# Corleno/Nonstationary_Multivariate_Gaussian_Process

Measured on AMD Instinct MI355X. Metric: log-posterior evals/sec (N=2048, D=3 nonseparable GP), higher is better.
Workload: dtype f64

## Files before the change

nonstationary_multivariate_gaussian_process_amd/csrc/nmgp_api.hip:

```cpp
#include <cstdarg>

#include "nmgp_internal.h"

using namespace nmgpk;

enum {
    SC_LOGDET = 0,
    SC_QUAD = 1,
    SC_PRIORQ = 2,
    SC_TRACE = 40,
    SC_OUT = 48,
    SC_MISC = 56,
    SC_COUNT = 128
};

int nmgp_fail(nmgp_ctx* ctx, int code, const char* fmt, ...) {
    char buf[1024];
    va_list ap;
    va_start(ap, fmt);
    vsnprintf(buf, sizeof(buf), fmt, ap);
    va_end(ap);
    if (ctx) ctx->err = buf;
    return code;
}
// ... 774 lines not shown
    PriorFactor pf;
    pf.alpha = alpha;
    pf.beta = beta;
    const size_t N = c->N, B = (size_t)c->batch / c->b_cps;
    pf.ld = (int)(((N + 15) / 16) * 16);
    NMGP_TRY(nmgp_dev_alloc(c, &pf.L, B * (size_t)pf.ld * N));
    if (nmgp_dev_alloc(c, &pf.logdet, B) != 0) {
        hipFree(pf.L);
        return NMGP_E_NOMEM;
    }
    int* info;
    HIP_TRY(c, hipMalloc((void**)&info, B * sizeof(int)));
    hipMemsetAsync(info, 0, B * sizeof(int), c->stream);
    rbf_cov_sym(c->stream, c->b_x, c->N, alpha, beta, pf.L, pf.ld, false, (int)B);
    nmgp_potrf(c, pf.L, pf.ld, c->N, 0, 0, info, (int)B, (long long)pf.ld * N, 1, 1);
    half_logdet(c->stream, pf.L, pf.ld, c->N, pf.logdet, (int)B);
    std::vector<int> hi(B);
    hipMemcpyAsync(hi.data(), info, B * sizeof(int), hipMemcpyDeviceToHost, c->stream);
    hipError_t e = hipStreamSynchronize(c->stream);
    hipFree(info);
    int bad = 0;
    for (size_t b = 0; b < B; ++b)
        if (hi[b] != 0 && bad == 0) bad = hi[b];
    if (e != hipSuccess || bad != 0) {
        hipFree(pf.L);
        hipFree(pf.logdet);
        if (e != hipSuccess) return nmgp_fail(c, NMGP_E_HIP, "batched prior factorisation failed (%s)", hipGetErrorString(e));
        return nmgp_fail(c, bad, "GP prior covariance RBF(alpha=%g, beta=%g)+jitter of a subject is not positive definite "
                         "(leading minor %d)", alpha, beta, bad);
    }
    c->b_priors.push_back(pf);
    *out = &c->b_priors.back();
    return 0;
}

static int batch_grad_alloc(nmgp_ctx* c) {
    if (c->b_grad_ready) return 0;
    const size_t N = c->N, T = c->T, n = c->n, P = (size_t)c->P_svc, B = c->batch;
    const size_t ld2 = nmgp_ld(2 * n + 2);
    const size_t NJ = (N + 63) / 64;
    NMGP_TRY(nmgp_dev_alloc(c, &c->b_S2, B * ld2 * n));
    NMGP_TRY(nmgp_dev_alloc(c, &c->b_Sinv, B * n * n));
    NMGP_TRY(nmgp_dev_alloc(c, &c->b_alpha, B * n));
    NMGP_TRY(nmgp_dev_alloc(c, &c->b_part, B * std::max(NJ * N * (T + 1), (size_t)n * ((n + 255) / 256))));
    NMGP_TRY(nmgp_dev_alloc(c, &c->b_grad, B * P));
    NMGP_TRY(nmgp_dev_alloc(c, &c->b_R2, N * B * (1 + T)));
    NMGP_TRY(nmgp_dev_alloc(c, &c->b_tr, B * 2));
    c->b_grad_ready = true;
    return 0;
}

static bool schur_selected(const nmgp_ctx* c, int want_grad) {
    if (want_grad || c->M < 2 || c->svc_schur == 0) return false;
    return true;
}

static int svc_batch_value_schur(nmgp_ctx* c, const double* xs, int xstride, const double* ys, long long ystride, int cps) {
    const int N = c->N, M = c->M, B = c->batch, n1 = (M - 1) * N;
    const long long P = c->P_svc;
    const int xpad = (N + 1) & 1, xoffA = N + 1 + xpad;
    const int ldA = (int)nmgp_ld((size_t)2 * N + 2), ldP = (int)nmgp_ld((size_t)n1 + 1);
    auto r64 = [](size_t v) { return (v + 63) / 64 * 64; };
    const size_t offP = r64((size_t)ldA * N), offPart = r64(offP + (size_t)ldP * n1);
    const size_t need = r64(offPart + (size_t)N * ((N + 255) / 256));
    const size_t bsS = nmgp_ld((size_t)c->n + 1) * (size_t)c->n;
    double* base = c->b_S;
    size_t bsz = bsS;
    if (need > bsS) {
        if (c->b_schur_stride != need) {
            NMGP_TRY(nmgp_dev_alloc(c, &c->b_schur, (size_t)B * need));
            c->b_schur_stride = need;
        }
        base = c->b_schur;
        bsz = need;
    }
    const long long bs = (long long)bsz;
    double* A = base;
    double* Sp = base + offP;
    double* part = base + offPart;
    double* w = c->b_z;
    double* w1 = c->b_z + (size_t)B * N;
    const double* tse = c->b_pars + (P - 1);
    hipStream_t s = c->stream;
    HIP_TRY(c, hipMemsetAsync(c->b_info2, 0, (size_t)B * sizeof(int), s));
    {
        StageScope sp(c, NMGP_STAGE_COV);
        svc_prep(s, c->b_pars, N, M, c->b_ell, c->b_Lv, B);
        int r = svc_schur_a(s, xs, c->b_ell, c->b_Lv, tse, ys, A, ldA, xpad, N, M, B, bs, xstride, ystride, cps);
        if (r) return nmgp_fail(c, r, "unsupported number of outputs M=%d", M);
    }
    {
        StageScope sp(c, NMGP_STAGE_CHOL);
        nmgp_potrf(c, A, ldA, N, 1 + xpad, N, c->b_info, B, bs, 1);
    }
    {
        StageScope sp(c, NMGP_STAGE_SOLVE);
        get_row(s, A, ldA, N, w, N, B, bs, N);
        tri_gemv_upper(s, A + xoffA, ldA, N, w, c->b_u, part, B, bs, bs);
    }
    {
        StageScope sp(c, NMGP_STAGE_REDUCE);
        chol_logdet_quad(s, A, ldA, N, w, c->b_scal + 2, c->b_scal + 3, B, bs, 16);
    }
    {
        StageScope sp(c, NMGP_STAGE_INVERSE);
        const SchurEpi e{xs, c->b_ell, c->b_Lv, tse, ys, c->b_u, Sp, ldP, N, xstride, cps, ystride, bs};
        int r = syrk_schur(s, A + xoffA, ldA, N, M, B, e);
        if (r) return nmgp_fail(c, r, "unsupported number of outputs M=%d", M);
    }
    {
        StageScope sp(c, NMGP_STAGE_CHOL);
        nmgp_potrf(c, Sp, ldP, n1, 1, 0, c->b_info2, B, bs, 1);
    }
    {
        StageScope sp(c, NMGP_STAGE_SOLVE);
        get_row(s, Sp, ldP, n1, w1, n1, B, bs, n1);
    }
    {
        StageScope sp(c, NMGP_STAGE_REDUCE);
        chol_logdet_quad(s, Sp, ldP, n1, w1, c->b_scal + 4, c->b_scal + 5, B, bs, 16);
        svc_schur_combine(s, c->b_Lv, N, M, c->b_scal, 16, c->b_info, c->b_info2, B);
    }
    return 0;
}

extern "C" int nmgp_svc_batch_eval(nmgp_ctx* c, const double hyper[8], int prior, int want_grad) {
    if (!c) return NMGP_E_NULL;
    if (!hyper) return nmgp_fail(c, NMGP_E_NULL, "hyper must not be NULL");
    if (c->batch <= 0) return nmgp_fail(c, NMGP_E_STATE, "nmgp_svc_batch_alloc must be called first");
    HIP_TRY(c, hipSetDevice(c->device));
    const int N = c->N, M = c->M, T = c->T, n = c->n, B = c->batch;
    const long long P = c->P_svc;
    c->b_traj_ready = false;
    if (want_grad) NMGP_TRY(batch_grad_alloc(c));
    const int xpad = (n + 1) & 1, xoff = n + 1 + xpad;
    const int ld = want_grad ? (int)nmgp_ld((size_t)2 * n + 2) : (int)nmgp_ld((size_t)n + 1);
    double* S = want_grad ? c->b_S2 : c->b_S;
    const long long bs = (long long)ld * n;
    const double mu_l = hyper[0], al_l = hyper[1], be_l = hyper[2], mu_L = hyper[3], al_L = hyper[4], be_L = hyper[5];
    const double a = hyper[6], b = hyper[7];
    hipStream_t s = c->stream;
    const bool multi = c->b_multi;
    const int cps = multi ? c->b_cps : 1;
    const double* xs = multi ? c->b_x : c->d_x;
    const int xstride = multi ? N : 0;
    PriorFactor *pl = nullptr, *pL = nullptr;
    if (multi) {
        NMGP_TRY(get_batch_prior(c, al_l, be_l, &pl));
        NMGP_TRY(get_batch_prior(c, al_L, be_L, &pL));
        NMGP_TRY(get_batch_prior(c, al_l, be_l, &pl));
    } else {
        NMGP_TRY(nmgp_get_prior(c, al_l, be_l, &pl));
        NMGP_TRY(nmgp_get_prior(c, al_L, be_L, &pL));
        NMGP_TRY(nmgp_get_prior(c, al_l, be_l, &pl));
    }
    HIP_TRY(c, hipMemsetAsync(c->b_info, 0, (size_t)B * sizeof(int), s));
    if (nmgp_poison()) HIP_TRY(c, hipMemsetAsync(c->b_scal, 0xFF, (size_t)B * 16 * sizeof(double), s));
    PriorStreamScope ps(c);
    if (schur_selected(c, want_grad)) {
        NMGP_TRY(svc_batch_value_schur(c, xs, xstride, multi ? c->b_y : c->d_y, multi ? n : 0, cps));
    } else {
        {
            StageScope sp(c, NMGP_STAGE_COV);
            svc_prep(s, c->b_pars, N, M, c->b_ell, c->b_Lv, B);
            int r = svc_cov_build(s, xs, c->b_ell, c->b_Lv, c->b_pars + (P - 1), S, ld, N, M, false, B, bs, xstride, cps);
            if (r) return nmgp_fail(c, r, "unsupported number of outputs M=%d", M);
        }
        {
            StageScope sp(c, NMGP_STAGE_CHOL);
            set_row(s, S, ld, n, multi ? c->b_y : c->d_y, n, B, bs, multi ? n : 0, cps);
            if (want_grad) identity_rows(s, S, ld, n + 1, n, xpad, B, bs);
            nmgp_potrf(c, S, ld, n, want_grad ? 1 + xpad : 1, want_grad ? n : 0, c->b_info, B, bs, 1);
        }
        {
            StageScope sp(c, NMGP_STAGE_SOLVE);
            get_row(s, S, ld, n, c->b_z, n, B, bs, n);
            if (want_grad) {
                tri_gemv_upper(s, S + xoff, (int)ld, n, c->b_z, c->b_alpha, c->b_part, (int)B, bs,
                               (long long)n * ((n + 255) / 256));
            }
        }
        {
            StageScope sp(c, NMGP_STAGE_REDUCE);
            chol_logdet_quad(s, S, ld, n, c->b_z, c->b_scal, c->b_scal + 1, B, bs, 16);
        }
    }
    {
        NmgpStage sp(c, NMGP_STAGE_PRIOR, ps.sp, 0.0, 0.0);
        const double one = 1.0;
// ... 810 lines not shown
```

nonstationary_multivariate_gaussian_process_amd/csrc/nmgp_chol.hip:

```cpp
#include "nmgp_internal.h"
#include <cstring>

namespace nmgpk {

static inline int cdiv_c(long long a, long long b) { return (int)((a + b - 1) / b); }

typedef double v4d __attribute__((ext_vector_type(4)));

#define SY_BM 128
#define SY_BK 16
#define SY_LD (SY_BM + 16)
#define SY_SB 8

__device__ __forceinline__ int clamp_row_pair(int r, int rows) {
    int rc = r < rows - 1 ? r : rows - 2;
    return rc < 0 ? 0 : rc;
}

__device__ __forceinline__ double fast_recip(double p) {
    double x = __builtin_amdgcn_rcp(p);
    double e = fma(-p, x, 1.0);
    x = fma(x, e, x);
    e = fma(-p, x, 1.0);
    x = fma(x, e, x);
// ... 115 lines not shown
                svc_schur_value<M>(sigma2, a, b, r == c, Lr, il2, Lc, kv, nai, gcb);
        }
    }
}

constexpr int svc_gstride(int M) { return M + 2; }

template <int M>
__device__ __forceinline__ void svc_schur_gtable(const SchurEpi& e, double* lds, int row0, int col0, int tid) {
    constexpr int T = M * (M + 1) / 2, GS = svc_gstride(M);
    if constexpr (M <= 4) {
        double* gt = lds + 8 * SCHUR_PATCH;
        if (tid < 256) {
            const int loc = tid < 128 ? col0 + tid : row0 + tid - 128;
            if (loc < e.N) {
                const double sigma2 = exp(e.tse[0]);
                const double* Lc = e.Lv + (size_t)loc * T;
                const double l00 = Lc[0];
#pragma unroll
                for (int b = 1; b < M; ++b) gt[tid * GS + b - 1] = sigma2 * Lc[b * (b + 1) / 2] / (l00 * l00);
                gt[tid * GS + M - 1] = 1.0 / (l00 * l00);
                gt[tid * GS + M] = e.x[loc];
                gt[tid * GS + M + 1] = e.ell[loc];
            }
        }
        __syncthreads();
    }
}

template <int M>
__device__ __forceinline__ void svc_schur_patch(const SchurEpi& e, double* P, const double* lds, int i0, int j0, int row0, int col0,
                                                int lane) {
    constexpr int T_ = M * (M + 1) / 2, GS = svc_gstride(M);
    constexpr int QU = M <= 3 ? 2 : 1;
    const int N = e.N;
    const size_t Ns = (size_t)N;
    const double sigma2 = exp(e.tse[0]);
    const double* gt = lds + 8 * SCHUR_PATCH;
    const int lo = lane & 31, hi = lane >> 5;
    __builtin_amdgcn_wave_barrier();
#pragma unroll
    for (int pass = 0; pass < 2; ++pass) {
        if (pass == 1 && M == 2) break;
        const int r = (pass == 0 ? i0 : j0) + lo;
        if (r < N) {
            const double* __restrict__ Lr = e.Lv + (size_t)r * T_;
            const double xr = e.x[r], lr = e.ell[r];
            const double xr2 = xr * xr, lr2 = lr * lr;
            const double l00 = Lr[0];
            const double il2 = 1.0 / (l00 * l00);
#pragma unroll QU
            for (int q = 0; q < 16; ++q) {
                const int o = 2 * q + hi;
                const int il = pass == 0 ? lo : o, jl = pass == 0 ? o : lo;
                const int c = (pass == 0 ? j0 : i0) + o;
                if (pass == 0 ? (c > r || c >= N) : (c <= r || c >= N)) continue;
                const double* gc = gt + (pass == 0 ? c - col0 : 128 + c - row0) * GS;
                if (pass == 1 && M == 3) {
                    e.S[(size_t)c * e.ld + (Ns + r)] = P[il * 33 + jl];
                    continue;
                }
                const double xc = M <= 4 ? gc[M] : e.x[c], lc = M <= 4 ? gc[M + 1] : e.ell[c];
                const double dist = (xr2 + xc * xc) - 2.0 * (xr * xc);
                const double Aa = lr2 + lc * lc;
                double kv = sqrt(2.0 * (lr * lc) / Aa) * exp(-dist / Aa);
                if (r == c) kv = NMGP_JITTER + kv;
                const double nai = P[il * 33 + jl];
                if (pass == 0) {
                    svc_schur_entries<M, true>(e, sigma2, r, Lr, il2, c, kv, nai, gc);
                    if (M == 3 && c < r) {
                        const double* Lc = e.Lv + (size_t)c * T_;
                        P[il * 33 + jl] = svc_schur_value<M>(sigma2, 2, 1, false, Lc, gc[M - 1], Lr, kv, nai, gt[(128 + r - row0) * GS]);
                    }
                } else {
                    svc_schur_entries<M, false>(e, sigma2, r, Lr, il2, c, kv, nai, gc);
                }
            }
        }
        __builtin_amdgcn_wave_barrier();
    }
}

template <int M>
__device__ __forceinline__ void svc_schur_yrow(const SchurEpi& e, int i) {
    constexpr int T = M * (M + 1) / 2;
    if (i >= e.N) return;
    const size_t Ns = (size_t)e.N;
    const int n1 = (M - 1) * e.N;
    const double sigma2 = exp(e.tse[0]);
    const double* Li = e.Lv + (size_t)i * T;
    const double l00 = Li[0];
    const double il2 = 1.0 / (l00 * l00);
    const double vi = e.y[i] / l00;
    const double r = vi - (sigma2 * il2) * e.u[i];
#pragma unroll
    for (int a = 1; a < M; ++a) e.S[((size_t)(a - 1) * Ns + i) * e.ld + n1] = e.y[(size_t)a * Ns + i] - Li[a * (a + 1) / 2] * r;
}

template <int SM = 0>
__device__ __forceinline__ void syrk_tile_fast(const double* __restrict__ A, int lda, double* __restrict__ C, int ldc, int K,
                                               int row0, int col0, bool diag, int kt0, bool beta0, int ncw, int yrow,
                                               int nyr, double* sA0, double* sB0, bool skip00 = false,
                                               int* __restrict__ finfo = nullptr, int fgoff = 0, bool mirror = false,
                                               int fresh0 = 0x7fffffff, const SchurEpi* se = nullptr) {
    constexpr int BK = 16;
    constexpr int SBUF = BK * SY_LD;
    const int tid = threadIdx.x, lane = tid & 63, w = tid >> 6;
    const int wi = w & 1, wj = w >> 1;
    const int l15 = lane & 15, l4 = lane >> 4;
    const int rp = tid & 63, cg = tid >> 6;
    const int offA = (cg * lda + row0 + 2 * rp) * 8, offB = (cg * lda + col0 + 2 * rp) * 8;
    const __amdgpu_buffer_rsrc_t rsrc = __builtin_amdgcn_make_buffer_rsrc((void*)A, 0, 0x7fffffff, 0x00020000);
    const int gstep = BK * lda * 8, ghalf = 8 * lda * 8;
    int soff = kt0 * gstep;
    const bool has_y = diag && yrow >= 0;
    const bool ywave = has_y && wi == 0 && wj >= 2;
    const int offY = ((tid & 15) * lda + yrow + (tid >> 4)) * 8;
    double* sY = sB0;
    v4i ra0, ra1, rb0, rb1;
    double ry = 0.0;
    auto gload = [&]() {
        ra0 = __builtin_amdgcn_raw_buffer_load_b128(rsrc, offA, soff, 0);
        ra1 = __builtin_amdgcn_raw_buffer_load_b128(rsrc, offA, soff + ghalf, 0);
        if (!diag) {
            rb0 = __builtin_amdgcn_raw_buffer_load_b128(rsrc, offB, soff, 0);
            rb1 = __builtin_amdgcn_raw_buffer_load_b128(rsrc, offB, soff + ghalf, 0);
        }
        if (has_y && tid < 16 * nyr) {
            typedef int v2i __attribute__((ext_vector_type(2)));
            const v2i t2 = __builtin_amdgcn_raw_buffer_load_b64(rsrc, offY, soff, 0);
            ry = __builtin_bit_cast(double, t2);
        }
        soff += gstep;
    };
    double* wA = sA0 + cg * SY_LD + 2 * rp;
    double* wB = sB0 + cg * SY_LD + 2 * rp;
    auto sstore = [&](int buf) {
        *reinterpret_cast<v4i*>(wA + buf * SBUF) = ra0;
        *reinterpret_cast<v4i*>(wA + buf * SBUF + 8 * SY_LD) = ra1;
        if (!diag) {
            *reinterpret_cast<v4i*>(wB + buf * SBUF) = rb0;
            *reinterpret_cast<v4i*>(wB + buf * SBUF + 8 * SY_LD) = rb1;
        }
        if (has_y && tid < 16 * nyr) sY[buf * 256 + tid] = ry;
    };
    const bool active = !(diag && (wi * 64 + 63 < wj * 32)) && (wj * 32 < ncw) && !(skip00 && wi == 0 && wj < 2);
    const int nk = K / BK;
    gload();
    v4d acc[2][2][2];
    if (active) {
        const int rw0 = __builtin_amdgcn_readfirstlane(row0 + wi * 64);
        const bool wload = !beta0 && rw0 < fresh0;
#pragma unroll
        for (int p = 0; p < 2; ++p) {
            const int i = row0 + wi * 64 + 32 * p + 2 * l15;
            const bool old = i < fresh0;
#pragma unroll
            for (int tj = 0; tj < 2; ++tj)
#pragma unroll
                for (int r = 0; r < 4; ++r) {
                    const int j = col0 + wj * 32 + 2 * (l4 + 4 * r) + tj;
                    double2 c = make_double2(0.0, 0.0);
                    if (wload && old) c = *reinterpret_cast<const double2*>(&C[(size_t)j * ldc + i]);
                    acc[p][0][tj][r] = -c.x;
                    acc[p][1][tj][r] = -c.y;
                }
        }
    }
    if (ywave) {
#pragma unroll
        for (int u = 0; u < 2; ++u)
#pragma unroll
            for (int t = 0; t < 2; ++t)
#pragma unroll
                for (int r = 0; r < 4; ++r) {
                    const int j = col0 + 64 * (wj - 2) + 32 * u + 2 * (l4 + 4 * r) + t;
                    acc[u][0][t][r] = (l15 < nyr && yrow + l15 < fresh0) ? -C[(size_t)j * ldc + yrow + l15] : 0.0;
                }
    }
    sstore(0);
    __syncthreads();
    const double* rA = sA0 + wi * 64 + 2 * l15 + l4 * SY_LD;
    const double* rB = (diag ? sA0 : sB0) + wj * 32 + 2 * l15 + l4 * SY_LD;
    auto compute = [&](int buf) {
        const double* tA = rA + buf * SBUF;
        const double* tB = rB + buf * SBUF;
        v2d fa[2], fb, na[2], nb;
        fa[0] = *reinterpret_cast<const v2d*>(tA);
        fa[1] = *reinterpret_cast<const v2d*>(tA + 32);
        fb = *reinterpret_cast<const v2d*>(tB);
#pragma unroll
        for (int kk = 0; kk < BK / 4; ++kk) {
            if (kk + 1 < BK / 4) {
                na[0] = *reinterpret_cast<const v2d*>(tA + (kk + 1) * 4 * SY_LD);
                na[1] = *reinterpret_cast<const v2d*>(tA + (kk + 1) * 4 * SY_LD + 32);
                nb = *reinterpret_cast<const v2d*>(tB + (kk + 1) * 4 * SY_LD);
            }
#pragma unroll
            for (int tj = 0; tj < 2; ++tj)
#pragma unroll
                for (int p = 0; p < 2; ++p)
#pragma unroll
                    for (int sx = 0; sx < 2; ++sx)
                        acc[p][sx][tj] = __builtin_amdgcn_mfma_f64_16x16x4f64(fb[tj], fa[p][sx], acc[p][sx][tj], 0, 0, 0);
            if (kk + 1 < BK / 4) {
                fa[0] = na[0];
                fa[1] = na[1];
                fb = nb;
            }
        }
    };
    const double* rY = sA0 + 64 * (wj - 2) + 2 * l15 + l4 * SY_LD;
    const int yz = (l15 < nyr) ? yrow + l15 - fresh0 - l4 : 0x7fffffff;
    auto compute_y = [&](int buf, int kb) {
        const double* tB = rY + buf * SBUF;
        const double* ty = sY + buf * 256 + l15 * 16 + l4;
#pragma unroll
        for (int kk = 0; kk < BK / 4; ++kk) {
            const v2d f0 = *reinterpret_cast<const v2d*>(tB + kk * 4 * SY_LD);
            const v2d f1 = *reinterpret_cast<const v2d*>(tB + kk * 4 * SY_LD + 32);
            const double yv = ty[4 * kk];
            const double fy = (kb + 4 * kk >= yz) ? yv : 0.0;
            acc[0][0][0] = __builtin_amdgcn_mfma_f64_16x16x4f64(f0[0], fy, acc[0][0][0], 0, 0, 0);
            acc[0][0][1] = __builtin_amdgcn_mfma_f64_16x16x4f64(f0[1], fy, acc[0][0][1], 0, 0, 0);
            acc[1][0][0] = __builtin_amdgcn_mfma_f64_16x16x4f64(f1[0], fy, acc[1][0][0], 0, 0, 0);
            acc[1][0][1] = __builtin_amdgcn_mfma_f64_16x16x4f64(f1[1], fy, acc[1][0][1], 0, 0, 0);
        }
    };
    for (int kt = kt0; kt < nk; kt += 2) {
        gload();
        if (active) compute(0);
        else if (ywave) compute_y(0, kt * BK);
        sstore(1);
        __syncthreads();
        if (kt + 2 < nk) gload();
        if (active) compute(1);
        else if (ywave) compute_y(1, kt * BK + BK);
        if (kt + 2 < nk) sstore(0);
        __syncthreads();
    }
    if constexpr (SM > 0) {
        svc_schur_gtable<SM>(*se, sA0, row0, col0, tid);
        if (active) {
            double* P = sA0 + w * SCHUR_PATCH;
#pragma unroll
            for (int p = 0; p < 2; ++p) {
#pragma unroll
                for (int sx = 0; sx < 2; ++sx)
#pragma unroll
                    for (int tj = 0; tj < 2; ++tj)
#pragma unroll
                        for (int r = 0; r < 4; ++r) P[(2 * l15 + sx) * 33 + 2 * (l4 + 4 * r) + tj] = -acc[p][sx][tj][r];
                svc_schur_patch<SM>(*se, P, sA0, row0 + wi * 64 + 32 * p, col0 + wj * 32, row0, col0, lane);
            }
        }
        if (diag && wj == 0) svc_schur_yrow<SM>(*se, row0 + wi * 64 + lane);
        return;
    }
    if (ywave && l15 < nyr) {
#pragma unroll
        for (int u = 0; u < 2; ++u)
#pragma unroll
            for (int t = 0; t < 2; ++t)
#pragma unroll
                for (int r = 0; r < 4; ++r) {
                    const int j = col0 + 64 * (wj - 2) + 32 * u + 2 * (l4 + 4 * r) + t;
                    C[(size_t)j * ldc + yrow + l15] = -acc[u][0][t][r];
                }
    }
    const bool fowner = finfo != nullptr && wi == 0 && wj < 2;
    if (active && !fowner) {
#pragma unroll
    for (int p = 0; p < 2; ++p)
#pragma unroll
        for (int tj = 0; tj < 2; ++tj)
#pragma unroll
            for (int r = 0; r < 4; ++r) {
                const int i = row0 + wi * 64 + 32 * p + 2 * l15;
                const int j = col0 + wj * 32 + 2 * (l4 + 4 * r) + tj;
                if (diag && j > i + 1) continue;
                double2 c;
                c.x = -acc[p][0][tj][r];
                c.y = -acc[p][1][tj][r];
                if (diag && j == i + 1) C[(size_t)j * ldc + i + 1] = c.y;
                else *reinterpret_cast<double2*>(&C[(size_t)j * ldc + i]) = c;
            }
    }
    if (mirror && active) {
        double* T = sA0 + w * (32 * 33);
        const int jl = lane & 31, ih = lane >> 5;
#pragma unroll
        for (int p = 0; p < 2; ++p) {
#pragma unroll
            for (int sx = 0; sx < 2; ++sx)
#pragma unroll
                for (int tj = 0; tj < 2; ++tj)
#pragma unroll
                    for (int r = 0; r < 4; ++r) T[(2 * l15 + sx) * 33 + 2 * (l4 + 4 * r) + tj] = -acc[p][sx][tj][r];
            const int rowm = col0 + wj * 32 + jl;
#pragma unroll
            for (int q = 0; q < 16; ++q) {
                const int il = 2 * q + ih;
                const int colm = row0 + wi * 64 + 32 * p + il;
                const double v = T[il * 33 + jl];
                if (colm > rowm) C[(size_t)colm * ldc + rowm] = v;
            }
        }
    }
    if (finfo != nullptr) syrk_fused_first_block(sA0, acc, fowner, wj, C, ldc, finfo, fgoff);
}

template <int NWJ, int BK, int SM = 0>
__device__ __forceinline__ void syrk_tile_body(const double* __restrict__ A, int lda, double* __restrict__ C, int ldc, int mrows,
                                               int ncols, int K, long long bstride, long long cstride, int ktri, int swz,
                                               int nbatch, int bx, int by, int bz0, double* sAb, double* sBb,
                                               int tri_row0 = 0x7fffffff, int tri_k0 = 0, int* __restrict__ finfo = nullptr,
                                               int fistride = 0, int fgoff = 0, const SchurEpi* sep = nullptr) {
    const int nyr = (ktri >> 2) & 31;
    const bool skipq = (ktri & 128) != 0;
    const bool mirror = (ktri & 512) != 0;
    const bool rowmajor = (ktri & 1024) != 0;
    const int yrow = nyr ? mrows : -1;
    (void)rowmajor;
    ktri &= 1;
    const int fresh0 = tri_row0 == 0x7fffffff ? 0x7fffffff : tri_row0 + tri_k0;
    constexpr int NT = 128 * NWJ;
    constexpr int CW = 128 / NWJ;
    constexpr int TJ = CW / 16;
    constexpr int NQ = (64 * BK) / NT;
    constexpr int CGS = NT / 64;
    double (*sA)[BK * SY_LD] = reinterpret_cast<double (*)[BK * SY_LD]>(sAb);
    double (*sB)[BK * SY_LD] = reinterpret_cast<double (*)[BK * SY_LD]>(sBb);
    int bi = bx, bj = by;
    int bz = bz0;
    if (swz) {
        const int t = bx, q = t >> 3;
        const int tiles_pm = swz > 0 ? swz : -swz;
        const long long g = swz > 0 ? ((long long)(q >> 6) * 8 + (t & 7)) * 64 + (q & 63) : (long long)t;
        int idx;
        if (finfo != nullptr) {
            if (g >= (long long)tiles_pm * nbatch) return;
            if (g < nbatch) {
                bz = (int)g;
                idx = 0;
            } else {
                const long long g2 = g - nbatch;
                bz = (int)(g2 / (tiles_pm - 1));
                idx = 1 + (int)(g2 - (long long)bz * (tiles_pm - 1));
            }
        } else {
            bz = (int)(g / tiles_pm);
            if (bz >= nbatch) return;
            idx = (int)(g - (long long)bz * tiles_pm);
        }
        const int gx = (mrows + SY_BM - 1) / SY_BM, gy = (ncols + SY_BM - 1) / SY_BM;
        if (rowmajor) {
            const int tri = gy * (gy + 1) / 2;
            if (idx < tri) {
                int b = (int)((sqrt(8.0 * (double)idx + 1.0) - 1.0) * 0.5);
                while ((b + 1) * (b + 2) / 2 <= idx) ++b;
                while (b * (b + 1) / 2 > idx) --b;
                bi = b;
                bj = idx - b * (b + 1) / 2;
            } else {
                bi = gy + (idx - tri) / gy;
                bj = (idx - tri) % gy;
            }
        } else {
        int c0 = 0, W = 0, cnt = 0;
        for (;; c0 += SY_SB) {
            W = gy - c0 < SY_SB ? gy - c0 : SY_SB;
            cnt = W * (W + 1) / 2 + (gx - c0 - W) * W;
            if (idx < cnt) break;
            idx -= cnt;
        }
        const int tri = W * (W + 1) / 2;
        if (idx < tri) {
            int b = 0;
            while (idx >= W - b) {
                idx -= W - b;
                ++b;
            }
            bj = c0 + b;
            bi = bj + idx;
        } else {
            idx -= tri;
            const int blk = idx / (SY_SB * W), in = idx - blk * (SY_SB * W);
            const int base = c0 + W + blk * SY_SB;
            const int rb = gx - base < SY_SB ? gx - base : SY_SB;
            bj = c0 + in / rb;
            bi = base + in % rb;
        }
        }
    }
    if (bi < bj) return;
    bi = __builtin_amdgcn_readfirstlane(bi);
    bj = __builtin_amdgcn_readfirstlane(bj);
    bz = __builtin_amdgcn_readfirstlane(bz);
    A += (size_t)bz * bstride;
    C += (size_t)bz * cstride;
    SchurEpi se{};
    if constexpr (SM > 0) {
        static_assert(NWJ == 4 && BK == 16, "the Schur epilogue assumes 8 waves of 64 x 32");
        constexpr int T = SM * (SM + 1) / 2;
        se = *sep;
        se.x += (size_t)(bz / se.cps) * se.xstride;
        se.y += (size_t)(bz / se.cps) * se.ystride;
        se.ell += (size_t)bz * se.N;
        se.Lv += (size_t)bz * se.N * T;
        se.tse += (size_t)bz * ((size_t)se.N * (1 + T) + 1);
        se.u += (size_t)bz * se.N;
        se.S += (size_t)bz * se.bstride;
    }
    const bool diag = (bi == bj);
    const int tid = threadIdx.x, lane = tid & 63, w = tid >> 6;
    const int wi = w & 1, wj = w >> 1;
    const int row0 = bi * SY_BM, col0 = bj * SY_BM;
    if constexpr (NWJ == 4 && BK == 16) {
        const int ncw = ncols - col0 >= SY_BM ? SY_BM : ncols - col0;
        if (row0 + SY_BM <= mrows && (ncw == SY_BM || ncw == 64) && col0 + SY_BM <= mrows && (K & 31) == 0 &&
            (long long)(K + 16) * lda * 8 < 0x7fff0000LL) {
            int kt0f = ktri ? row0 / BK : 0;
            if (row0 >= tri_row0) {
                const int z = (row0 - tri_row0 - tri_k0) / BK;
                kt0f = z > 0 ? (z & ~1) : 0;
            }
            syrk_tile_fast<SM>(A, lda, C, ldc, K, row0, col0, diag, kt0f, ktri != 0, ncw, yrow, nyr, &sA[0][0], &sB[0][0],
                               skipq && bi == 0 && bj == 0, (finfo != nullptr && bi == 0 && bj == 0) ? finfo + (size_t)bz * fistride : nullptr,
                               fgoff, mirror, fresh0, &se);
            return;
        }
    }
    const int rp = tid & 63, cg = tid >> 6;
    double2 ra[NQ], rb[NQ];

    const int ri = row0 + 2 * rp, rj = col0 + 2 * rp;
    const int ric = clamp_row_pair(ri, mrows), rjc = clamp_row_pair(rj, mrows);
    const bool ix = ri < mrows, iy = ri + 1 < mrows, jx = rj < mrows, jy = rj + 1 < mrows;
    const bool ish = ix && (ric != ri), jsh = jx && (rjc != rj);
    auto gload = [&](int k0) {
#pragma unroll
        for (int q = 0; q < NQ; ++q) {
            const int kc = k0 + cg + CGS * q;
            const double* colp = A + (size_t)(kc < K ? kc : K - 1) * lda;
            ra[q] = *reinterpret_cast<const double2*>(colp + ric);
            if (!diag) rb[q] = *reinterpret_cast<const double2*>(colp + rjc);
        }
    };
    auto sstore = [&](int buf, int k0) {
#pragma unroll
        for (int q = 0; q < NQ; ++q) {
            const int kl = cg + CGS * q;
            const bool kin = (k0 + kl) < K;
            double2 va, vb;
            va.x = (kin && ix) ? (ish ? ra[q].y : ra[q].x) : 0.0;
            va.y = (kin && iy) ? ra[q].y : 0.0;
            *reinterpret_cast<double2*>(&sA[buf][kl * SY_LD + 2 * rp]) = va;
            if (!diag) {
                vb.x = (kin && jx) ? (jsh ? rb[q].y : rb[q].x) : 0.0;
                vb.y = (kin && jy) ? rb[q].y : 0.0;
                *reinterpret_cast<double2*>(&sB[buf][kl * SY_LD + 2 * rp]) = vb;
            }
        }
    };

    const bool active = !(diag && (wi * 64 + 63 < wj * CW));
    const bool skip00g = skipq && bi == 0 && bj == 0;
    const int nk = (K + BK - 1) / BK;
    int kt0 = ktri ? (row0 / BK) : 0;
    if (row0 >= tri_row0 && row0 - tri_row0 - tri_k0 > 0) kt0 = (row0 - tri_row0 - tri_k0) / BK;
    gload(kt0 * BK);
    v4d acc[TJ][4];
#pragma unroll
    for (int tj = 0; tj < TJ; ++tj)
#pragma unroll
        for (int ti = 0; ti < 4; ++ti)
#pragma unroll
            for (int r = 0; r < 4; ++r) {
                const int i = row0 + wi * 64 + ti * 16 + (lane & 15);
                const int j = col0 + wj * CW + tj * 16 + (lane >> 4) + 4 * r;
                acc[tj][ti][r] = (!ktri && active && i < mrows && j < ncols && i >= j) ? C[(size_t)j * ldc + i] : 0.0;
            }
    if (row0 + SY_BM > fresh0) {
#pragma unroll
        for (int tj = 0; tj < TJ; ++tj)
#pragma unroll
            for (int ti = 0; ti < 4; ++ti)
#pragma unroll
                for (int r = 0; r < 4; ++r)
                    acc[tj][ti][r] = (row0 + wi * 64 + ti * 16 + (lane & 15) >= fresh0) ? 0.0 : acc[tj][ti][r];
    }
    sstore(0, kt0 * BK);
    __syncthreads();
    for (int kt = kt0; kt < nk; ++kt) {
        const int cur = (kt - kt0) & 1;
        if (kt + 1 < nk) gload((kt + 1) * BK);
        if (active) {
            const double* tA = sA[cur] + wi * 64 + (lane & 15) + (lane >> 4) * SY_LD;
            const double* tB = (diag ? sA[cur] : sB[cur]) + wj * CW + (lane & 15) + (lane >> 4) * SY_LD;
            double fa[4], fb[TJ], na[4], nb[TJ];
#pragma unroll
            for (int t = 0; t < 4; ++t) fa[t] = tA[t * 16];
#pragma unroll
            for (int t = 0; t < TJ; ++t) fb[t] = -tB[t * 16];
#pragma unroll
            for (int kk = 0; kk < BK / 4; ++kk) {
                if (kk + 1 < BK / 4) {
#pragma unroll
                    for (int t = 0; t < 4; ++t) na[t] = tA[(kk + 1) * 4 * SY_LD + t * 16];
#pragma unroll
                    for (int t = 0; t < TJ; ++t) nb[t] = -tB[(kk + 1) * 4 * SY_LD + t * 16];
                }
#pragma unroll
                for (int tj = 0; tj < TJ; ++tj)
#pragma unroll
                    for (int ti = 0; ti < 4; ++ti)
                        acc[tj][ti] = __builtin_amdgcn_mfma_f64_16x16x4f64(fb[tj], fa[ti], acc[tj][ti], 0, 0, 0);
                if (kk + 1 < BK / 4) {
#pragma unroll
                    for (int t = 0; t < 4; ++t) fa[t] = na[t];
#pragma unroll
                    for (int t = 0; t < TJ; ++t) fb[t] = nb[t];
                }
            }
        }
        if (kt + 1 < nk) sstore(cur ^ 1, (kt + 1) * BK);
        __syncthreads();
    }
    if constexpr (SM > 0) {
        svc_schur_gtable<SM>(se, sAb, row0, col0, tid);
        if (active) {
            double* P = sAb + w * SCHUR_PATCH;
#pragma unroll
            for (int h = 0; h < 2; ++h) {
#pragma unroll
                for (int tj = 0; tj < TJ; ++tj)
#pragma unroll
                    for (int t2 = 0; t2 < 2; ++t2)
#pragma unroll
                        for (int r = 0; r < 4; ++r)
                            P[(t2 * 16 + (lane & 15)) * 33 + tj * 16 + (lane >> 4) + 4 * r] = acc[tj][2 * h + t2][r];
                svc_schur_patch<SM>(se, P, sAb, row0 + wi * 64 + 32 * h, col0 + wj * CW, row0, col0, lane);
            }
        }
        if (diag && wj == 0) svc_schur_yrow<SM>(se, row0 + wi * 64 + lane);
        return;
    }
    if (active) {
#pragma unroll
        for (int tj = 0; tj < TJ; ++tj)
#pragma unroll
            for (int ti = 0; ti < 4; ++ti)
#pragma unroll
                for (int r = 0; r < 4; ++r) {
                    const int i = row0 + wi * 64 + ti * 16 + (lane & 15);
                    const int j = col0 + wj * CW + tj * 16 + (lane >> 4) + 4 * r;
                    if (i < mrows && j < ncols && i >= j && !(skip00g && i < 64 && j < 64)) C[(size_t)j * ldc + i] = acc[tj][ti][r];
                    if (mirror && i < mrows && j < ncols && i > j) C[(size_t)i * ldc + j] = acc[tj][ti][r];
                }
    }
}

__global__ __launch_bounds__(512, 4) void k_syrk_lower(const double* __restrict__ A, int lda, double* __restrict__ C, int ldc,
                                                        int mrows, int ncols, int K, long long bstride, long long cstride,
                                                        int ktri, int swz, int nbatch, int tri_row0, int tri_k0,
                                                        int* __restrict__ finfo, int fistride, int fgoff) {
    __shared__ __attribute__((aligned(16))) double smem[4 * SY_BK * SY_LD];
    syrk_tile_body<4, SY_BK>(A, lda, C, ldc, mrows, ncols, K, bstride, cstride, ktri, swz, nbatch, blockIdx.x, blockIdx.y,
                             blockIdx.z, smem, smem + 2 * SY_BK * SY_LD, tri_row0, tri_k0, finfo, fistride, fgoff);
}

template <int M>
__global__ __launch_bounds__(512, 4) void k_syrk_schur(const double* __restrict__ A, int lda, int N, long long bstride, int kflags,
                                                        int swz, int nbatch, SchurEpi se) {
    __shared__ __attribute__((aligned(16))) double smem[SY_SCHUR_SMEM];
    syrk_tile_body<4, SY_BK, M>(A, lda, nullptr, 0, N, N, N, bstride, 0, kflags, swz, nbatch, blockIdx.x, blockIdx.y, blockIdx.z,
                                smem, smem + 2 * SY_BK * SY_LD, 0x7fffffff, 0, nullptr, 0, 0, &se);
}

struct Switches {
    enum Panel { kAuto, kFused, kRec, kRl };
    Panel panel = kAuto;
    int fused_max_batch = -1;
    int fused_base = 0;
    int la_max_batch = 16;
    int syrk_small_max = 256;
    const char* step_stamps = nullptr;
};
static const Switches& switches() {
    static const Switches sw = [] {
        Switches w;
        if (const char* e = std::getenv("NMGP_CHOL_PANEL"))
            w.panel = std::strcmp(e, "fused") == 0 ? Switches::kFused
                      : std::strcmp(e, "rec") == 0 ? Switches::kRec : std::strcmp(e, "rl") == 0 ? Switches::kRl : Switches::kAuto;
        if (const char* e = std::getenv("NMGP_CHOL_FUSED_MAX_BATCH")) w.fused_max_batch = std::atoi(e);
        if (const char* e = std::getenv("NMGP_CHOL_FUSED_BASE")) w.fused_base = (std::atoi(e) / 64) * 64;
        if (const char* e = std::getenv("NMGP_CHOL_LA_MAX_BATCH")) w.la_max_batch = std::atoi(e);
        if (const char* e = std::getenv("NMGP_SYRK_SMALL_MAX")) w.syrk_small_max = std::atoi(e);
        w.step_stamps = std::getenv("NMGP_STEP_STAMPS");
        return w;
    }();
    return sw;
}

struct StepStamps {
    long long* dev = nullptr;
    int cap = 0;
    long long* begin(hipStream_t s, int nsteps) {
        if (!switches().step_stamps) return nullptr;
        if (cap < nsteps) {
            if (dev) hipFree(dev);
            if (hipMalloc((void**)&dev, (size_t)nsteps * 16 * sizeof(long long)) != hipSuccess) dev = nullptr;
            cap = dev ? nsteps : 0;
        }
        if (dev) hipMemsetAsync(dev, 0, (size_t)cap * 16 * sizeof(long long), s);
        return dev;
    }
    void dump(hipStream_t s, int nsteps) const {
        if (!switches().step_stamps || !dev) return;
        std::vector<long long> h((size_t)nsteps * 16);
        hipStreamSynchronize(s);
        hipMemcpy(h.data(), dev, h.size() * sizeof(long long), hipMemcpyDeviceToHost);
        if (FILE* f = std::fopen(switches().step_stamps, "w")) {
            for (int k = 0; k < nsteps; ++k) {
                for (int j = 0; j < 9; ++j) std::fprintf(f, "%lld ", h[(size_t)k * 16 + j]);
                std::fprintf(f, "\n");
            }
            std::fclose(f);
// ... 376 lines not shown
        __syncthreads();
        if (kt + 1 >= nk) break;
        compute(1);
        if (kt + 2 < nk) {
            sstore(ra[0], rb[0], 0, (kt + 2) * 16);
            if (kt + 4 < nk) gload(ra[0], rb[0], (kt + 4) * 16);
        }
        __syncthreads();
    }
    if (info != nullptr && bi == 0 && bj == 0) {
        Potf2Lds& P = *reinterpret_cast<Potf2Lds*>(smem);
#pragma unroll
        for (int k = 0; k < 16; ++k) {
            const int idx = tid + 256 * k;
            const int r = idx & 63, c = idx >> 6;
            if (c > r) P.S[c * PB_LD + r] = 0.0;
        }
        if (active) {
#pragma unroll
            for (int tj = 0; tj < 2; ++tj)
#pragma unroll
                for (int ti = 0; ti < 2; ++ti)
#pragma unroll
                    for (int r = 0; r < 4; ++r) {
                        const int i = wi * 32 + ti * 16 + l15;
                        const int j = wj * 32 + tj * 16 + l4 + 4 * r;
                        if (i >= j) P.S[j * PB_LD + i] = acc[tj][ti][r];
                    }
        }
        __syncthreads();
        potf2b_core_mfma(P, info + (size_t)bz * istride, goff);
        potf2b_store(C, ldc, 64, P, tid, 256);
        return;
    }
    if (active) {
#pragma unroll
        for (int tj = 0; tj < 2; ++tj)
#pragma unroll
            for (int ti = 0; ti < 2; ++ti)
#pragma unroll
                for (int r = 0; r < 4; ++r) {
                    const int i = row0 + wi * 32 + ti * 16 + l15;
                    const int j = col0 + wj * 32 + tj * 16 + l4 + 4 * r;
                    if (i < mrows && j < ncols && i >= j) C[(size_t)j * ldc + i] = acc[tj][ti][r];
                }
    }
}

bool syrk_lower(hipStream_t s, const double* A, int lda, double* C, int ldc, int mrows, int ncols, int K, int batch,
                long long bstride, long long cstride, int ktri, int tri_row0, int tri_k0, int* finfo, int fistride, int goff,
                const SyrkHook* hook) {
    if (mrows <= 0 || ncols <= 0 || K <= 0) return false;
    const SyrkPlan pl = syrk_plan(lda, ldc, mrows, ncols, K, batch, ktri, false, tri_row0 != kNoTriRows);
    const long long cs = cstride < 0 ? bstride : cstride;
    void* tok = nullptr;
    if (hook && hook->begin) {
        const double elems = (double)ncols * mrows - 0.5 * (double)ncols * (ncols - 1);
        tok = hook->begin(hook->user, s, 2.0 * K * elems * batch, 8.0 * batch * (2.0 * elems + (double)mrows * K));
    }
    bool fused;
    if (!ktri && K >= 128 && batch <= 16 && (long long)pl.tiles * batch <= switches().syrk_small_max && cs == bstride &&
        (lda & 1) == 0 && mrows >= 2) {
        const int gx = (mrows + 63) / 64, gy = (ncols + 63) / 64;
        int tiles = 0;
        for (int bj = 0; bj < gy; ++bj) tiles += gx - bj > 0 ? gx - bj : 0;
        fused = finfo != nullptr && mrows >= 64 && ncols >= 64;
        NMGP_LAUNCH(k_syrk_small, dim3((unsigned)(tiles * batch)), dim3(256), 0, s, A, lda, C, ldc, mrows, ncols, K, bstride, tiles,
                    batch, tri_row0, tri_k0, fused ? finfo : (int*)nullptr, fistride, goff);
    } else {
        fused = finfo != nullptr && !ktri && cs == bstride && pl.mrows >= SY_BM && (ncols >= SY_BM || ncols == 64) &&
                (K & 31) == 0 && (long long)(K + 16) * lda * 8 < 0x7fff0000LL;
        SyrkPlan pf = pl;
        if (fused && pf.swz == 0) {
            pf.grid = dim3((unsigned)((long long)pf.tiles * batch), 1, 1);
            pf.swz = -pf.tiles;
        }
        NMGP_LAUNCH(k_syrk_lower, pf.grid, dim3(512), 0, s, A, lda, C, ldc, pf.mrows, ncols, K, bstride, cs, pf.kflags,
                    pf.swz, batch, tri_row0, tri_k0, fused ? finfo : (int*)nullptr, fistride, goff);
    }
    if (tok && hook->end) hook->end(hook->user, tok);
    return fused;
}

int syrk_schur(hipStream_t s, const double* X, int lda, int N, int M, int batch, const SchurEpi& e) {
    if (N <= 0) return 0;
    if (M < 2 || M > 8) return NMGP_E_UNSUPPORTED;
    const SyrkPlan pl = syrk_plan(lda, lda, N, N, N, batch, 2, false);
    switch (M) {
#define SCHUR_CASE(m) \
        case m: NMGP_LAUNCH(k_syrk_schur<m>, pl.grid, dim3(512), 0, s, X, lda, pl.mrows, e.bstride, pl.kflags, pl.swz, batch, e); break;
        SCHUR_CASE(2) SCHUR_CASE(3) SCHUR_CASE(4) SCHUR_CASE(5) SCHUR_CASE(6) SCHUR_CASE(7) SCHUR_CASE(8)
#undef SCHUR_CASE
    }
    return 0;
}


template <int SRC>
__device__ inline double quad_bcast(double v) {
    constexpr int ctrl = SRC | (SRC << 2) | (SRC << 4) | (SRC << 6);
    int lo = __double2loint(v), hi = __double2hiint(v);
    lo = __builtin_amdgcn_mov_dpp(lo, ctrl, 0xF, 0xF, true);
    hi = __builtin_amdgcn_mov_dpp(hi, ctrl, 0xF, 0xF, true);
    return __hiloint2double(hi, lo);
}

template <int KC, int GC>
__device__ __forceinline__ void trsm_step(double (&x)[16], const double (*Lm)[65], const double* rinv, int g) {
    constexpr int c = 4 * KC + GC;
    double xc = x[KC] * rinv[c];
    xc = quad_bcast<GC>(xc);
    if (g == GC) x[KC] = xc;
    double t[16];
#pragma unroll
    for (int kk = KC; kk < 16; ++kk) t[kk] = Lm[4 * kk + g][c];
    {
        const double upd = x[KC] - xc * t[KC];
        x[KC] = (g > GC) ? upd : x[KC];
    }
#pragma unroll
    for (int kk = KC + 1; kk < 16; ++kk) x[kk] -= xc * t[kk];
}

template <int KC>
__device__ __forceinline__ void trsm_steps4(double (&x)[16], const double (*Lm)[65], const double* rinv, int g) {
    trsm_step<KC, 0>(x, Lm, rinv, g);
    trsm_step<KC, 1>(x, Lm, rinv, g);
    trsm_step<KC, 2>(x, Lm, rinv, g);
    trsm_step<KC, 3>(x, Lm, rinv, g);
}

__global__ __launch_bounds__(256) void k_trsm_64(const double* __restrict__ L, int ldl, int nb, double* __restrict__ A,
                                                  int lda, int rows, long long bstride) {
    L += (size_t)blockIdx.y * bstride;
    A += (size_t)blockIdx.y * bstride;
    __shared__ double Lm[64][65];
    __shared__ double rinv[64];
    const int tid = threadIdx.x;
    const int lr = tid >> 2, g = tid & 3;
    const int row = blockIdx.x * 64 + lr;
    const bool valid = row < rows;
    double x[16], lv[16];
#pragma unroll
    for (int kk = 0; kk < 16; ++kk) {
        const int k = 4 * kk + g;
        x[kk] = (valid && k < nb) ? A[(size_t)k * lda + row] : 0.0;
    }
#pragma unroll
    for (int q = 0; q < 16; ++q) {
        const int idx = tid + 256 * q;
        const int r = idx & 63, c = idx >> 6;
        double v = (r == c) ? 1.0 : 0.0;
        if (r < nb && c <= r) v = L[(size_t)c * ldl + r];
        lv[q] = v;
    }
#pragma unroll
    for (int q = 0; q < 16; ++q) {
        const int idx = tid + 256 * q;
        Lm[idx & 63][idx >> 6] = lv[q];
    }
    __syncthreads();
    if (tid < 64) rinv[tid] = 1.0 / Lm[tid][tid];
    __syncthreads();
    trsm_steps4<0>(x, Lm, rinv, g);   trsm_steps4<1>(x, Lm, rinv, g);   trsm_steps4<2>(x, Lm, rinv, g);
    trsm_steps4<3>(x, Lm, rinv, g);   trsm_steps4<4>(x, Lm, rinv, g);   trsm_steps4<5>(x, Lm, rinv, g);
    trsm_steps4<6>(x, Lm, rinv, g);   trsm_steps4<7>(x, Lm, rinv, g);   trsm_steps4<8>(x, Lm, rinv, g);
    trsm_steps4<9>(x, Lm, rinv, g);   trsm_steps4<10>(x, Lm, rinv, g);  trsm_steps4<11>(x, Lm, rinv, g);
    trsm_steps4<12>(x, Lm, rinv, g);  trsm_steps4<13>(x, Lm, rinv, g);  trsm_steps4<14>(x, Lm, rinv, g);
    trsm_steps4<15>(x, Lm, rinv, g);
#pragma unroll
// ... 665 lines not shown
```

nonstationary_multivariate_gaussian_process_amd/csrc/nmgp_internal.h:

```cpp
#pragma once

#include <hip/hip_runtime.h>
#include <rocblas/rocblas.h>
#include <rocsolver/rocsolver.h>

#include <cmath>
#include <cstdio>
#include <cstdlib>
#include <cstring>
#include <map>
#include <string>
#include <utility>
#include <vector>

#include "nmgp.h"

#define NMGP_JITTER 1e-6
#define NMGP_PRECISION 1e-6

struct DevBuf {
    double* p = nullptr;
    size_t cap = 0;
};

// ... 302 lines not shown
                const double* Sinv, int ld, int N, int M, double* part, double ssign = 1.0, int batch = 1,
                int xstride = 0, int cps = 1);
#define NMGP_XTRI_SEED_BLOCKS 3
#define NMGP_TRI_GEMV_BLOCK 256
void tri_gemv_upper(hipStream_t s, const double* W, int ld, int n, const double* z, double* out, double* part, int batch = 1,
                    long long wstride = 0, long long pstride = 0);
void trace_terms(hipStream_t s, const double* alpha, const double* Sinv, int ld, int n, double* out,
                 double ssign = 1.0, int batch = 1);
void svc_grad_final(hipStream_t s, const double* part, int NJ, int N, int M, const double* Lv, const double* R2,
                    int ldR, const double* pars, const double* tr, double a, double b, int prior, double* grad,
                    int batch = 1);
void svc_finalize(hipStream_t s, const double* logdet, const double* quad, const double* q, const double* hl_l,
                  const double* hl_L, const double* pars, long long P, int N, int T, double a, double b,
                  double ig_const, int prior, double* out5, int batch = 1, int sstride = 0, int hstride = 0, int cps = 1);
void half_logdet(hipStream_t s, const double* L, int ld, int n, double* out, int batch = 1);
int kron_mv(hipStream_t s, const double* K, int n1, int n2, const double* y, const double* B, int m1, int m2,
            double* out);
void eig_reduce(hipStream_t s, double* a, const double* wB, int M, const double* wK, int N, const double* sigma2p,
                bool scale, double* out);
void colscale_d(hipStream_t s, const double* V, const double* wB, int M, const double* wK, int N, const double* sigma2p,
                double* Vs);
void colscale(hipStream_t s, const double* V, const double* svec, int rows, int cols, double* Vs);
void sep_coreB(hipStream_t s, const double* At, const double* wB, int M, const double* wK, int N,
               const double* sigma2p, double* coreB);
void sep_adjoint(hipStream_t s, const double* x, const double* ell, const double* sig, const double* U,
                 const double* wB, int M, const double* C, int N, double* part);
void sep_grad_sum(hipStream_t s, const double* part, int NJ, int N, double* g);
void exp_vec(hipStream_t s, const double* in, int n, double* out);
void fill_vec(hipStream_t s, double* out, int n, double v);
void two_col_rhs(hipStream_t s, const double* a, double mu_a, const double* b, double mu_b, int N, double* R);
void sub_vec(hipStream_t s, const double* y, const double* mu, int n, double* out);
void dot(hipStream_t s, const double* a, const double* b, int n, double* out);
void kron_eigvec(hipStream_t s, const double* VB, int M, const double* VK, int N, double* U);
void kron_w(hipStream_t s, const double* wB, int M, const double* wK, int N, double sigma2, double* w);
void svc_star(hipStream_t st, const double* proj, int S, int M, double mu_l, double mu_L, double* tl_star,
              double* Lstar);
void svc_crosscov_rows(hipStream_t st, const double* x, const double* ell, const double* Lv, int N, int M, const double* xs,
                       const double* tl_star, const double* Lstar, int S, double* A, int ld, int R0);
void pred_rows_reduce(hipStream_t st, const double* A, int ld, int n, int R0, int zrow, int E, double* part, double* mean,
                      double* colsq);
void svc_predvar(hipStream_t st, const double* Lstar, const double* colsq, int S, int M, const double* tse,
                 double* var);
void sep_crossvec(hipStream_t st, int mode, const double* x, const double* sig, const double* ell, int N,
                  const double* xs, const double* tl_star, const double* ts_star, double sig0, double l0, int S,
                  double* KX);
void sep_predict(hipStream_t st, const double* Cq, const double* a, const double* wB, const double* VB, int M,
                 const double* wK, int N, double sigma2, const double* Bdiag, const double* kss, bool strict_clip, int S,
                 double* mean, double* var);
void sep_predict_chol(hipStream_t st, const double* dots, const double* sqs, const double* wB, const double* VB, int M, double sigma2,
                      const double* Bdiag, const double* kss, bool strict_clip, int S, double* mean, double* var);
void cols_to_rows(hipStream_t st, const double* KX, int N, int S, double* A, int ld, int R0, int batch, long long bstride);
void sep_star(hipStream_t st, const double* proj, int S, double mu_l, double mu_s, double* tl_star, double* ts_star,
              double* kss);
void add_diag(hipStream_t s, double* A, int ld, int n, double v);
void rotate_y(hipStream_t s, const double* Y, const double* VB, int N, int M, double* yt);
void sep_blocks(hipStream_t s, const double* K, const double* wB, const double* sigma2p, int N, int M, double* out,
                int ldo, long long bstride);
#define NMGP_SEP_TR_G 128
int sep_traces(hipStream_t s, const double* Cneg, const double* K, const double* alpha, int N, int M, double* out);
void weighted_sum_lower(hipStream_t s, const double* Cneg, const double* wB, int N, int M, double* C);
void sep_prep_b(hipStream_t s, const double* pars, long long P, const double* Y, const double* small, int small_per, int N, int M,
                double* ell, double* sig, double* yt, int B);
void sep_blocks_b(hipStream_t s, const double* x, const double* ell, const double* sig, const double* small, int small_per, int N, int M,
                  double* S, int ldo, long long bstride, double* Kout, int B);
void sep_reduce_b(hipStream_t s, const double* Cneg, const double* K, const double* alpha, const double* small, int small_per, int N,
                  int M, int G, double* C, double* out, double* xi, int B);
void sep_adjoint_b(hipStream_t s, const double* x, const double* ell, const double* sig, const double* U, const double* small,
                   int small_per, int M, const double* C, int N, double* part, double* g, int B);
void two_col_rhs_b(hipStream_t s, const double* pars, long long P, double mu_a, double mu_b, int N, double* R, int B);
void ps_rows_reduce(hipStream_t s, const double* A, int ld, long long bstride, int n, int R0, int zrow, int E, double* part,
                    int batch, double* dots, double* sqs, long long ostride, long long o0);
void pss_star(hipStream_t s, const double* W0, const double* W1, const double* cv0, const double* cv1, const double* pars, long long P,
              const double* z, int N, int S, double mu_l, double mu_s, double* star, int B);
bool syrk_lower(hipStream_t s, const double* A, int lda, double* C, int ldc, int mrows, int ncols, int K, int batch,
                long long bstride, long long cstride = -1, int ktri = 0, int tri_row0 = 0x7fffffff, int tri_k0 = 0,
                int* finfo = nullptr, int fistride = 0, int goff = 0, const SyrkHook* hook = nullptr);
struct SchurEpi {
    const double* x;
    const double* ell;
    const double* Lv;
    const double* tse;
    const double* y;
    const double* u;
    double* S;
    int ld;
    int N;
    int xstride;
    int cps;
    long long ystride;
    long long bstride;
};
int syrk_schur(hipStream_t s, const double* X, int lda, int N, int M, int batch, const SchurEpi& e);
void identity_rows(hipStream_t s, double* A, int lda, int row0, int n, int pad, int batch = 1, long long bstride = 0);
void set_row(hipStream_t s, double* A, int lda, int row, const double* v, int n, int batch, long long bstride,
             long long vstride, int cps = 1);
void get_row(hipStream_t s, const double* A, int lda, int row, double* v, int n, int batch, long long bstride,
             long long vstride);
void potrf_lower(hipStream_t s, hipStream_t s2, hipEvent_t* ev, double* A, int lda, int n, int extra, int xtri,
                 int nb1, int* info, int batch, long long bstride, int istride, const SyrkHook* hook = nullptr,
                 int precise = 0);

}
```

Baseline: 1693.

## Fuse triangular gemv for u into Schur SYRK kernel's idle y-waves

When the shape allows it, the separate upper-triangular gemv that computes u is skipped. The idle y-waves in the Schur SYRK diagonal tiles instead accumulate the dot products of the factor columns with the row w, reading w directly from matrix A. The result is staged in shared memory and used by the y-row epilogue. This removes one kernel launch and one pass over the triangular factor, in exchange for more complexity in the SYRK kernel and an extra barrier for large M.

```diff
diff --git a/nonstationary_multivariate_gaussian_process_amd/csrc/nmgp_api.hip b/nonstationary_multivariate_gaussian_process_amd/csrc/nmgp_api.hip
--- a/nonstationary_multivariate_gaussian_process_amd/csrc/nmgp_api.hip
+++ b/nonstationary_multivariate_gaussian_process_amd/csrc/nmgp_api.hip
@@ -880,6 +880,7 @@
     double* w1 = c->b_z + (size_t)B * N;
     const double* tse = c->b_pars + (P - 1);
     hipStream_t s = c->stream;
+    const bool fuse_u = syrk_schur_fuses_u(ldA, N);
     HIP_TRY(c, hipMemsetAsync(c->b_info2, 0, (size_t)B * sizeof(int), s));
     {
         StageScope sp(c, NMGP_STAGE_COV);
@@ -894,7 +895,7 @@
     {
         StageScope sp(c, NMGP_STAGE_SOLVE);
         get_row(s, A, ldA, N, w, N, B, bs, N);
-        tri_gemv_upper(s, A + xoffA, ldA, N, w, c->b_u, part, B, bs, bs);
+        if (!fuse_u) tri_gemv_upper(s, A + xoffA, ldA, N, w, c->b_u, part, B, bs, bs);
     }
     {
         StageScope sp(c, NMGP_STAGE_REDUCE);
@@ -902,7 +903,7 @@
     }
     {
         StageScope sp(c, NMGP_STAGE_INVERSE);
-        const SchurEpi e{xs, c->b_ell, c->b_Lv, tse, ys, c->b_u, Sp, ldP, N, xstride, cps, ystride, bs};
+        const SchurEpi e{xs, c->b_ell, c->b_Lv, tse, ys, c->b_u, fuse_u ? A + N : nullptr, Sp, ldP, N, xstride, cps, ystride, bs};
         int r = syrk_schur(s, A + xoffA, ldA, N, M, B, e);
         if (r) return nmgp_fail(c, r, "unsupported number of outputs M=%d", M);
     }
diff --git a/nonstationary_multivariate_gaussian_process_amd/csrc/nmgp_chol.hip b/nonstationary_multivariate_gaussian_process_amd/csrc/nmgp_chol.hip
--- a/nonstationary_multivariate_gaussian_process_amd/csrc/nmgp_chol.hip
+++ b/nonstationary_multivariate_gaussian_process_amd/csrc/nmgp_chol.hip
@@ -221,7 +221,7 @@
 }
 
 template <int M>
-__device__ __forceinline__ void svc_schur_yrow(const SchurEpi& e, int i) {
+__device__ __forceinline__ void svc_schur_yrow(const SchurEpi& e, int i, double ui) {
     constexpr int T = M * (M + 1) / 2;
     if (i >= e.N) return;
     const size_t Ns = (size_t)e.N;
@@ -231,7 +231,7 @@
     const double l00 = Li[0];
     const double il2 = 1.0 / (l00 * l00);
     const double vi = e.y[i] / l00;
-    const double r = vi - (sigma2 * il2) * e.u[i];
+    const double r = vi - (sigma2 * il2) * ui;
 #pragma unroll
     for (int a = 1; a < M; ++a) e.S[((size_t)(a - 1) * Ns + i) * e.ld + n1] = e.y[(size_t)a * Ns + i] - Li[a * (a + 1) / 2] * r;
 }
@@ -254,7 +254,10 @@
     int soff = kt0 * gstep;
     const bool has_y = diag && yrow >= 0;
     const bool ywave = has_y && wi == 0 && wj >= 2;
-    const int offY = ((tid & 15) * lda + yrow + (tid >> 4)) * 8;
+    const int offY = SM > 0 ? (tid & 15) * lda * 8
+                            : ((tid & 15) * lda + yrow + (tid >> 4)) * 8;
+    const __amdgpu_buffer_rsrc_t rsrcY =
+        __builtin_amdgcn_make_buffer_rsrc((void*)(SM > 0 && has_y ? se->w : A), 0, 0x7fffffff, 0x00020000);
     double* sY = sB0;
     v4i ra0, ra1, rb0, rb1;
     double ry = 0.0;
@@ -267,7 +270,7 @@
         }
         if (has_y && tid < 16 * nyr) {
             typedef int v2i __attribute__((ext_vector_type(2)));
-            const v2i t2 = __builtin_amdgcn_raw_buffer_load_b64(rsrc, offY, soff, 0);
+            const v2i t2 = __builtin_amdgcn_raw_buffer_load_b64(rsrcY, offY, soff, 0);
             ry = __builtin_bit_cast(double, t2);
         }
         soff += gstep;
@@ -306,7 +309,7 @@
                 }
         }
     }
-    if (ywave) {
+    if (SM == 0 && ywave) {
 #pragma unroll
         for (int u = 0; u < 2; ++u)
 #pragma unroll
@@ -366,20 +369,38 @@
             acc[1][0][1] = __builtin_amdgcn_mfma_f64_16x16x4f64(f1[1], fy, acc[1][0][1], 0, 0, 0);
         }
     };
+    double u0 = 0.0, u1 = 0.0;
+    auto compute_u = [&](int buf) {
+        const double* ta = sA0 + buf * SBUF + 64 * (wj - 2) + lane;
+        const double* tw = sY + buf * 256;
+#pragma unroll
+        for (int k = 0; k < BK; k += 2) {
+            u0 = fma(ta[k * SY_LD], tw[k], u0);
+            u1 = fma(ta[(k + 1) * SY_LD], tw[k + 1], u1);
+        }
+    };
     for (int kt = kt0; kt < nk; kt += 2) {
         gload();
         if (active) compute(0);
-        else if (ywave) compute_y(0, kt * BK);
+        else if (ywave) {
+            if constexpr (SM > 0) compute_u(0);
+            else compute_y(0, kt * BK);
+        }
         sstore(1);
         __syncthreads();
         if (kt + 2 < nk) gload();
         if (active) compute(1);
-        else if (ywave) compute_y(1, kt * BK + BK);
+        else if (ywave) {
+            if constexpr (SM > 0) compute_u(1);
+            else compute_y(1, kt * BK + BK);
+        }
         if (kt + 2 < nk) sstore(0);
         __syncthreads();
     }
     if constexpr (SM > 0) {
+        if (ywave) sA0[w * SCHUR_PATCH + lane] = u0 + u1;
         svc_schur_gtable<SM>(*se, sA0, row0, col0, tid);
+        if (SM > 4 && has_y) __syncthreads();
         if (active) {
             double* P = sA0 + w * SCHUR_PATCH;
 #pragma unroll
@@ -393,7 +414,10 @@
                 svc_schur_patch<SM>(*se, P, sA0, row0 + wi * 64 + 32 * p, col0 + wj * 32, row0, col0, lane);
             }
         }
-        if (diag && wj == 0) svc_schur_yrow<SM>(*se, row0 + wi * 64 + lane);
+        if (diag && wj == 0) {
+            const int i = row0 + wi * 64 + lane;
+            svc_schur_yrow<SM>(*se, i, has_y ? sA0[(4 + 2 * wi) * SCHUR_PATCH + lane] : se->u[i]);
+        }
         return;
     }
     if (ywave && l15 < nyr) {
@@ -549,6 +573,7 @@
         se.Lv += (size_t)bz * se.N * T;
         se.tse += (size_t)bz * ((size_t)se.N * (1 + T) + 1);
         se.u += (size_t)bz * se.N;
+        if (se.w) se.w += (size_t)bz * bstride;
         se.S += (size_t)bz * se.bstride;
     }
     const bool diag = (bi == bj);
@@ -682,7 +707,7 @@
                 svc_schur_patch<SM>(se, P, sAb, row0 + wi * 64 + 32 * h, col0 + wj * CW, row0, col0, lane);
             }
         }
-        if (diag && wj == 0) svc_schur_yrow<SM>(se, row0 + wi * 64 + lane);
+        if (diag && wj == 0 && row0 + wi * 64 + lane < se.N) svc_schur_yrow<SM>(se, row0 + wi * 64 + lane, se.u[row0 + wi * 64 + lane]);
         return;
     }
     if (active) {
@@ -1225,10 +1250,18 @@
     return fused;
 }
 
+bool syrk_schur_fuses_u(int lda, int N) {
+    return N > 0 && N % SY_BM == 0 && (lda & 1) == 0 && (long long)(N + 16) * lda * 8 < 0x7fff0000LL;
+}
+
 int syrk_schur(hipStream_t s, const double* X, int lda, int N, int M, int batch, const SchurEpi& e) {
     if (N <= 0) return 0;
     if (M < 2 || M > 8) return NMGP_E_UNSUPPORTED;
-    const SyrkPlan pl = syrk_plan(lda, lda, N, N, N, batch, 2, false);
+    SyrkPlan pl = syrk_plan(lda, lda, N, N, N, batch, 2, false);
+    if (e.w) {
+        if (!syrk_schur_fuses_u(lda, N)) return NMGP_E_UNSUPPORTED;
+        pl.kflags |= 1 << 2;
+    }
     switch (M) {
 #define SCHUR_CASE(m) \
         case m: NMGP_LAUNCH(k_syrk_schur<m>, pl.grid, dim3(512), 0, s, X, lda, pl.mrows, e.bstride, pl.kflags, pl.swz, batch, e); break;
diff --git a/nonstationary_multivariate_gaussian_process_amd/csrc/nmgp_internal.h b/nonstationary_multivariate_gaussian_process_amd/csrc/nmgp_internal.h
--- a/nonstationary_multivariate_gaussian_process_amd/csrc/nmgp_internal.h
+++ b/nonstationary_multivariate_gaussian_process_amd/csrc/nmgp_internal.h
@@ -408,6 +408,7 @@
     const double* tse;
     const double* y;
     const double* u;
+    const double* w;
     double* S;
     int ld;
     int N;
@@ -416,6 +417,7 @@
     long long ystride;
     long long bstride;
 };
+bool syrk_schur_fuses_u(int lda, int N);
 int syrk_schur(hipStream_t s, const double* X, int lda, int N, int M, int batch, const SchurEpi& e);
 void identity_rows(hipStream_t s, double* A, int lda, int row0, int n, int pad, int batch = 1, long long bstride = 0);
 void set_row(hipStream_t s, double* A, int lda, int row, const double* v, int n, int batch, long long bstride,
```

After: 1708 (median of 6 runs). About the same (+0.9%).
